# adamchang2000/DenseFusion

Measured on AMD Instinct MI355X. Metric: poses/sec (node) YCB-Video 1000 pts + 2 refine iters, higher is better.
Workload: dtype f32

## Files before the change

densefusion_amd/_lib.py:

```python
from __future__ import annotations

import ctypes
import os

_HERE = os.path.dirname(os.path.abspath(__file__))
LIB_PATH = os.path.join(_HERE, "libdfusion_hip_dev.so" if os.environ.get("DF_DEV_LIB") else "libdfusion_hip.so")
_lib = None

_vp, _i, _i64, _f, _sz = ctypes.c_void_p, ctypes.c_int, ctypes.c_int64, ctypes.c_float, ctypes.c_size_t

class ConvDesc(ctypes.Structure):
    _fields_ = ([(n, ctypes.c_void_p) for n in ("in_", "wgt", "bias", "res", "prelu", "out")] +
                [(n, ctypes.c_int32) for n in ("B", "H", "W", "Cin", "in_ld", "in_coff", "OH", "OW", "Cout", "out_ld",
                                               "out_coff", "res_ld", "res_coff", "KH", "KW", "stride", "pad", "dil",
                                               "act")] +
                [("splitk_ws", ctypes.c_void_p), ("splitk_ws_bytes", ctypes.c_size_t)])


SIGNATURES = {
    "df_last_error": (ctypes.c_char_p, []),
    "df_version": (_i, []),
    "df_knn_device": (_i, [_vp, _i, _vp, _i, _i, _i, _vp, _vp]),
    "df_knn": (_i, [_vp, _vp, _vp, _i, _i, _i, _i, _i, _vp]),
    "knn_device": (None, [_vp, _i, _vp, _i, _i, _i, _vp, _vp, _vp]),
# ... 55 lines not shown
    "df_trainer_flat_numel": (_i64, [_vp]),
    "df_trainer_num_params": (_i, [_vp]),
    "df_trainer_param_info": (_i, [_vp, _i, ctypes.c_char_p, _i, ctypes.POINTER(_i64), ctypes.POINTER(_i)]),
    "df_trainer_pack_param": (_i, [_vp, ctypes.c_char_p, _vp, _vp, _vp]),
    "df_trainer_unpack_param": (_i, [_vp, ctypes.c_char_p, _vp, _vp, _vp]),
    "df_posenet_train_workspace_bytes": (_sz, [_vp, _i, _i, _i, _i]),
    "df_posenet_train_step": (_i, [_vp, _vp, _vp, _i64, _i, _i, _i] + [_vp] * 6 + [_i, _vp, _f, _i, ctypes.c_uint] + [_vp] * 9 + [_sz, _vp]),
    "df_posenet_train_multi_workspace_bytes": (_sz, [_vp, _i, _vp, _vp, _vp, _i]),
    "df_posenet_train_step_multi": (_i, [_vp, _vp, _vp, _i64, _i, _vp, _vp, _vp, _vp] + [_vp] * 5 + [_i, _vp, _f, _i, ctypes.c_uint] + [_vp] * 9 + [_sz, _vp]),
    "df_trainer_set_splitk": (_i, [_vp, _i]),
    "df_trainer_profile": (_i, [_vp, _i]),
    "df_trainer_profile_read": (_i, [_vp, ctypes.POINTER(ctypes.c_double), ctypes.POINTER(ctypes.c_double), ctypes.POINTER(_i)]),
    "df_refiner_train_workspace_bytes": (_sz, [_vp, _i, _i]),
    "df_refiner_train_step": (_i, [_vp, _vp, _vp, _i64, _i] + [_vp] * 5 + [_i, _vp] + [_vp] * 4 + [_sz, _vp]),
    "df_conv3x3_winograd_tile_scratch_bytes": (ctypes.c_size_t, [ctypes.POINTER(ConvDesc), _i]),
    "df_conv3x3_winograd_tile_nhwc": (_i, [ctypes.POINTER(ConvDesc), _i, _vp, ctypes.c_size_t, _vp]),
    "df_conv2d_dgrad_nhwc": (_i, [ctypes.POINTER(ConvDesc), _vp, _vp, _vp, _i, _vp]),
    "df_conv2d_wgrad_workspace_bytes": (ctypes.c_size_t, [ctypes.POINTER(ConvDesc)]),
    "df_conv2d_wgrad_nhwc": (_i, [ctypes.POINTER(ConvDesc), _vp, _vp, _vp, _vp, ctypes.c_size_t, _vp]),
    "df_net_debug_taps": (_i, [_vp, _i]),
    "df_net_debug_tap_read": (_i, [_vp, ctypes.c_char_p, _vp, _i64, ctypes.POINTER(_i64)]),
    "df_net_profile": (_i, [_vp, _i]),
    "df_net_profile_read": (_i, [_vp] + [ctypes.POINTER(ctypes.c_double)] * 4 + [ctypes.POINTER(_i)]),
}


def lib():
    global _lib
    if _lib is None:
        if not os.path.exists(LIB_PATH):
            raise RuntimeError(
                f"{LIB_PATH} not found: the HIP extension is not built. Run "
                "`python -c 'import __graft_entry__ as g; g.build()'` at the repo root (needs hipcc). "
                "densefusion_amd has no CPU fallback.")
        L = ctypes.CDLL(LIB_PATH)
        for name, (res, args) in SIGNATURES.items():
            fn = getattr(L, name)
            fn.restype, fn.argtypes = res, args
        _lib = L
    return _lib


def check(status: int, what: str = "") -> None:
    if status != 0:
        msg = lib().df_last_error().decode("utf-8", "replace")
        raise RuntimeError(f"libdfusion_hip {what} failed ({status}): {msg}")
# ... 36 lines not shown
```

densefusion_amd/csrc/engine.hip:

```cpp
#include <cstdlib>
#include <cstring>
#include <map>
#include <string>
#include <vector>

#include "igemm.h"
#include "layers.h"
#include "wino.h"
#include "pose.h"

namespace df {

struct ParamInfo {
  std::string key;
  int64_t shape[4];
  int ndim;
  int64_t numel() const { int64_t n = 1; for (int i = 0; i < ndim; ++i) n *= shape[i]; return n; }
};

struct Net {
  int kind = 0;
  int num_points = 0, num_obj = 0;
  std::vector<ParamInfo> spec;
  std::map<std::string, int> index;
  std::vector<char> loaded;
  std::map<std::string, float *> buf;
  int device = 0;
  bool profiling = false;
  std::vector<hipEvent_t> ev;
  std::vector<double> ev_flops, ev_bytes, ev_useful;
  std::vector<std::string> ev_desc;
  size_t ev_used = 0;
  bool psp_dirty = false;
  bool upload_pending = false;
  float *stage = nullptr;
  size_t stage_cap = 0;
  bool taps_on = false;
  struct Tap { float *buf = nullptr; size_t cap = 0; int64_t shape[4] = {0, 0, 0, 0}; };
  std::map<std::string, Tap> taps;
};

static void add(Net &n, const std::string &key, std::initializer_list<int64_t> shp) {
  ParamInfo p;
  p.key = key;
  p.ndim = (int)shp.size();
  int i = 0;
  for (auto v : shp) p.shape[i++] = v;
  for (; i < 4; ++i) p.shape[i] = 1;
  n.index[key] = (int)n.spec.size();
  n.spec.push_back(p);
}

static const char *CNN = "cnn.model.module.";

static void build_posenet_spec(Net &n) {
// ... 175 lines not shown
    const std::string nm = std::string("fc") + std::to_string(l);
    if (ends_with(key, ".weight")) e = copy(dev_alloc(n, nm + ".w", (size_t)2 * co * ci) + (size_t)h * co * ci, src, (size_t)co * ci);
    else e = copy(dev_alloc(n, nm + ".bias", 2 * co) + h * co, src, co);
  } else {
    float *dst = dev_alloc(n, key, (size_t)numel);
    if (!dst) return set_error(DF_ERR_LAUNCH, "load_param: hipMalloc failed");
    e = copy(dst, src, (size_t)numel);
  }
  if (e == hipSuccess && n.kind == 1 && key == "feat.conv5.weight") {
    const float *w5 = n.buf[key];
    float *wx = dev_alloc(n, "feat.conv5.wx", (size_t)512 * 192), *we = dev_alloc(n, "feat.conv5.we", (size_t)512 * 192);
    if (!wx || !we) return set_error(DF_ERR_LAUNCH, "load_param: hipMalloc failed");
    e = copy2d(wx, 192, w5, 384, 64, 512);
    if (e == hipSuccess) e = copy2d(wx + 64, 192, w5 + 128, 384, 128, 512);
    if (e == hipSuccess) e = copy2d(we, 192, w5 + 64, 384, 64, 512);
    if (e == hipSuccess) e = copy2d(we + 64, 192, w5 + 256, 384, 128, 512);
  }
  if (e != hipSuccess) return set_error(DF_ERR_LAUNCH, "load_param(%s): %s", key.c_str(), hipGetErrorString(e));
  n.loaded[it->second] = 1;
  if (n.kind == 0 && key.find(".psp.") != std::string::npos && !ends_with(key, ".bias")) n.psp_dirty = true;
  return DF_OK;
}

static int ensure_derived(Net &n) {
  if (!n.psp_dirty) {
    if (n.upload_pending) {
      if (hipStreamSynchronize(0) != hipSuccess) return set_error(DF_ERR_LAUNCH, "parameter upload failed: %s", hipGetErrorString(hipGetLastError()));
      n.upload_pending = false;
    }
    return DF_OK;
  }
  const std::string P = CNN;
  float *wc = dev_alloc(n, "psp.fold.w", (size_t)4 * 1024 * 512), *wf = dev_alloc(n, "psp.fold.wfeat", (size_t)1024 * 512);
  if (!wc || !wf) return set_error(DF_ERR_LAUNCH, "psp fold: hipMalloc failed");
  const float *wb = n.buf[P + "psp.bottleneck.weight"];
  hipMemcpy2DAsync(wf, 512 * sizeof(float), wb + 2048, 2560 * sizeof(float), 512 * sizeof(float), 1024, hipMemcpyDeviceToDevice, 0);
  for (int st = 0; st < 4; ++st)
    hipLaunchKernelGGL(psp_fold_kernel, dim3(2, 1024, 1), dim3(256), 0, 0, wb, n.buf[P + "psp.stages." + std::to_string(st) + ".1.weight"], wc, st);
  if (hipStreamSynchronize(0) != hipSuccess || check_launch("psp fold") != DF_OK) return DF_ERR_LAUNCH;
  n.psp_dirty = false;
  n.upload_pending = false;
  return DF_OK;
}

static int check_ready(const Net &n0) {
  Net &n = const_cast<Net &>(n0);
  for (size_t i = 0; i < n.spec.size(); ++i)
    if (!n.loaded[i]) return set_error(DF_ERR_STATE, "parameter '%s' was never loaded", n.spec[i].key.c_str());
  return ensure_derived(n);
}

struct Ctx {
  Net *net;
  hipStream_t st;
  bool dry;
  char *base;
  size_t off = 0, cap = 0, peak = 0;
  int err = DF_OK;

  float *f(size_t floats) { return reinterpret_cast<float *>(bytes(floats * sizeof(float))); }
  void *bytes(size_t b) {
    b = (b + 255) & ~size_t(255);
    void *p = dry ? nullptr : base + off;
    off += b;
    if (off > peak) peak = off;
// ... 15 lines not shown
    const size_t n = (size_t)d0 * d1 * d2 * d3;
    if (t.cap < n) {
      if (t.buf) hipFree(t.buf);
      t.buf = nullptr; t.cap = 0;
      if (hipMalloc(&t.buf, n * sizeof(float)) != hipSuccess) { (void)hipGetLastError(); return; }
      t.cap = n;
    }
    t.shape[0] = d0; t.shape[1] = d1; t.shape[2] = d2; t.shape[3] = d3;
    hipMemcpyAsync(t.buf, src, n * sizeof(float), hipMemcpyDeviceToDevice, st);
  }
  double pt_useful = 1.0;
  void pconv(const ConvParams &p) { conv(p, pt_useful); }
  void conv(const ConvParams &p, double useful = 1.0) {
    if (!live()) return;
    Net &n = *net;
    if (n.profiling) {
      if (n.ev_used + 2 > n.ev.size()) {
        const size_t old = n.ev.size();
        n.ev.resize(old + 256);
        for (size_t i = old; i < n.ev.size(); ++i) hipEventCreate(&n.ev[i]);
      }
      hipEventRecord(n.ev[n.ev_used], st);
    }
#ifdef DF_DEV
    ConvParams pc = p;
    pc.wgt_const = true;
    const int rc = launch_conv(pc, st);
#else
    const int rc = launch_conv(p, st);
#endif
    if (n.profiling) {
      hipEventRecord(n.ev[n.ev_used + 1], st);
      n.ev_flops.push_back(conv_flops(p));
      n.ev_bytes.push_back(conv_bytes(p));
      n.ev_useful.push_back(conv_flops(p) * useful);
      char d[160];
      snprintf(d, sizeof(d), "M=%ld N=%d K=%d k%dx%d s%d d%d z%d", (long)p.B * p.OH * p.OW, p.Cout, p.KH * p.KW * p.Cin, p.KH,
               p.KW, p.stride, p.dil, p.zcount);
      n.ev_desc.push_back(d);
      n.ev_used += 2;
    }
    if (rc != DF_OK) err = rc;
  }
};

static ConvParams point_gemm(const float *in, int in_ld, int in_coff, int cin, const float *w, const float *bias,
                             float *out, int out_ld, int out_coff, int cout, int rows, int act);

static bool point_fused() {
  static const bool on = df::dev_getenv("DF_POINT_UNFUSED") == nullptr;
  return on;
}

static int wino_route_for(int H, int W, int dil, int ci, int co) {
  static const bool off = df::dev_getenv("DF_NO_WINOGRAD") != nullptr;
  static const int force = df::dev_getenv("DF_WINOGRAD_TILE") ? atoi(df::dev_getenv("DF_WINOGRAD_TILE")) : 0;
  if (off) return 0;
  const int r = wino_route(H, W, dil, ci, co);
  return (r && force == 2) ? 2 : r;
}

static ConvParams point_gemm(const float *in, int in_ld, int in_coff, int cin, const float *w, const float *bias,
// ... 369 lines not shown
extern "C" df_net *df_posenet_create(int num_points, int num_obj) {
  if (num_points <= 0 || num_obj <= 0) { set_error(DF_ERR_ARG, "posenet_create: bad sizes"); return nullptr; }
  Net *n = new Net();
  n->kind = 0; n->num_points = num_points; n->num_obj = num_obj;
  hipGetDevice(&n->device);
  build_posenet_spec(*n);
  n->loaded.assign(n->spec.size(), 0);
  return reinterpret_cast<df_net *>(n);
}

extern "C" df_net *df_refiner_create(int num_points, int num_obj) {
  if (num_points <= 0 || num_obj <= 0) { set_error(DF_ERR_ARG, "refiner_create: bad sizes"); return nullptr; }
  Net *n = new Net();
  n->kind = 1; n->num_points = num_points; n->num_obj = num_obj;
  hipGetDevice(&n->device);
  build_refiner_spec(*n);
  n->loaded.assign(n->spec.size(), 0);
  return reinterpret_cast<df_net *>(n);
}

extern "C" void df_net_destroy(df_net *h) {
  if (!h) return;
  Net *n = as_net(h);
#ifdef DF_DEV
  split_gemm_invalidate();
#endif
  for (auto &kv : n->buf) hipFree(kv.second);
  if (n->stage) hipFree(n->stage);
  for (auto &kv : n->taps) if (kv.second.buf) hipFree(kv.second.buf);
  for (auto e : n->ev) hipEventDestroy(e);
  delete n;
}

extern "C" int df_net_num_params(const df_net *h) { return h ? (int)as_net(h)->spec.size() : 0; }

extern "C" int df_net_param_info(const df_net *h, int i, char *key_out, int key_cap, int64_t *shape4, int *ndim) {
  if (!h) return set_error(DF_ERR_ARG, "param_info: null handle");
  const Net *n = as_net(h);
  if (i < 0 || i >= (int)n->spec.size()) return set_error(DF_ERR_ARG, "param_info: index out of range");
  const ParamInfo &p = n->spec[i];
  if (key_out && key_cap > 0) { strncpy(key_out, p.key.c_str(), key_cap - 1); key_out[key_cap - 1] = 0; }
  if (shape4) for (int d = 0; d < 4; ++d) shape4[d] = p.shape[d];
  if (ndim) *ndim = p.ndim;
  return DF_OK;
}

extern "C" int df_net_load_param(df_net *h, const char *key, const float *ptr, int64_t numel) {
  if (!h || !key) return set_error(DF_ERR_ARG, "load_param: null handle/key");
#ifdef DF_DEV
  split_gemm_invalidate();
#endif
  return load_param(*as_net(h), key, ptr, numel);
}

extern "C" int df_net_profile(df_net *h, int enable) {
  if (!h) return set_error(DF_ERR_ARG, "profile: null handle");
  Net *n = as_net(h);
  n->profiling = enable != 0;
  n->ev_used = 0;
  n->ev_flops.clear();
  n->ev_bytes.clear();
  n->ev_useful.clear();
  n->ev_desc.clear();
  return DF_OK;
}

extern "C" int df_net_profile_read(df_net *h, double *gemm_ms, double *gemm_flops, double *gemm_useful_flops, double *gemm_bytes,
                                   int *launches) {
  if (!h) return set_error(DF_ERR_ARG, "profile_read: null handle");
  Net *n = as_net(h);
  double ms = 0, fl = 0, by = 0, us = 0;
  static const bool verbose = df::dev_getenv("DF_PROFILE_VERBOSE") != nullptr;
  for (size_t i = 0; i + 1 < n->ev_used; i += 2) {
    float t = 0;
    if (hipEventElapsedTime(&t, n->ev[i], n->ev[i + 1]) != hipSuccess) return set_error(DF_ERR_LAUNCH, "profile_read: events not complete");
    ms += t;
    fl += n->ev_flops[i / 2];
    by += n->ev_bytes[i / 2];
    us += n->ev_useful[i / 2];
    if (verbose)
      fprintf(stderr, "[df-gemm] %s  %.1f us  %.1f TFLOP/s\n", n->ev_desc[i / 2].c_str(), t * 1e3, n->ev_flops[i / 2] / t / 1e9);
  }
  if (gemm_ms) *gemm_ms = ms;
  if (gemm_flops) *gemm_flops = fl;
  if (gemm_useful_flops) *gemm_useful_flops = us;
  if (gemm_bytes) *gemm_bytes = by;
  if (launches) *launches = (int)(n->ev_used / 2);
  n->ev_used = 0;
  n->ev_flops.clear();
  n->ev_bytes.clear();
  n->ev_useful.clear();
  n->ev_desc.clear();
  return DF_OK;
}

extern "C" int df_net_debug_taps(df_net *h, int enable) {
  if (!h) return set_error(DF_ERR_ARG, "debug_taps: null handle");
  Net *n = as_net(h);
  n->taps_on = enable != 0;
  if (!enable) {
    for (auto &kv : n->taps) if (kv.second.buf) hipFree(kv.second.buf);
    n->taps.clear();
  }
  return DF_OK;
}

extern "C" int df_net_debug_tap_read(df_net *h, const char *name, float *dst, int64_t cap, int64_t *shape4) {
  if (!h || !name) return set_error(DF_ERR_ARG, "debug_tap_read: null handle / name");
  Net *n = as_net(h);
  auto it = n->taps.find(name);
  if (it == n->taps.end() || !it->second.buf) return set_error(DF_ERR_STATE, "debug_tap_read: no tap named '%s' (arm df_net_debug_taps and run a single-bucket forward)", name);
  const Net::Tap &t = it->second;
  const int64_t numel = t.shape[0] * t.shape[1] * t.shape[2] * t.shape[3];
  if (shape4) for (int i = 0; i < 4; ++i) shape4[i] = t.shape[i];
  if (!dst) return DF_OK;
  if (cap < numel) return set_error(DF_ERR_ARG, "debug_tap_read: destination holds %lld floats, tap '%s' has %lld", (long long)cap, name, (long long)numel);
  if (hipMemcpy(dst, t.buf, (size_t)numel * sizeof(float), hipMemcpyDefault) != hipSuccess) return set_error(DF_ERR_LAUNCH, "debug_tap_read: copy failed");
// ... 355 lines not shown
```

densefusion_amd/csrc/igemm.h:

```cpp
#pragma once
#include "common.h"

namespace df {

enum Act { ACT_NONE = 0, ACT_RELU = 1, ACT_PRELU = 2 };

struct ConvParams {
  const float *in = nullptr;
  const float *wgt = nullptr;
  const float *bias = nullptr;
  const float *res = nullptr;
  const float *prelu = nullptr;
  float *out = nullptr;
  float *colsum = nullptr;
  int B = 1, H = 1, W = 1, Cin = 0, in_ld = 0, in_coff = 0;
  int OH = 1, OW = 1, Cout = 0, out_ld = 0, out_coff = 0;
  int res_ld = 0, res_coff = 0;
  int KH = 1, KW = 1, stride = 1, pad = 0, dil = 1;
  int up = 1;
  int act = ACT_NONE;
  int rows_per_group = 0, rows_valid = 0, bias_group_ld = 0;
  int zcount = 1;
  int ngroup = 0;
  long z_in_coff = 0, z_wgt = 0, z_bias = 0, z_out_coff = 0;
  bool wgt_const = false;
  float *splitk_ws = nullptr;
  size_t splitk_ws_bytes = 0;
  int splitk = 1;
  int tiles_m = 0, tile_gn = 0, tile_full = 0;
  unsigned full_magic = 0, gn_magic = 0, gl_magic = 0, rpg_magic = 0;
  int full_sh = 0, gn_sh = 0, gl_sh = 0, rpg_sh = 0;
  unsigned ohw_magic = 0, ow_magic = 0;
  int ohw_sh = 0, ow_sh = 0;
};

int conv_colsum_rows(const ConvParams &p);
double conv_flops(const ConvParams &p);
double conv_bytes(const ConvParams &p);
int launch_conv(const ConvParams &p, hipStream_t st, int *splitk_used = nullptr);

struct WgradSeg { int B, H, W, OH, OW; long in_row0, out_row0; };
constexpr int CONV_MAX_BUCKETS = 16;
int launch_conv_multi(const ConvParams &p, int nseg, const WgradSeg *segs, hipStream_t st);

size_t wgrad_workspace_bytes(const ConvParams &p);
int launch_wgrad(const ConvParams &p, float *dw, float *db, void *ws, size_t ws_bytes, hipStream_t st, int accumulate = 0);

constexpr int WGRAD_MAX_SEGS = 32;
size_t wgrad_multi_workspace_bytes(const ConvParams &p, int nseg, const WgradSeg *segs);
int launch_wgrad_multi(const ConvParams &p, int nseg, const WgradSeg *segs, float *dw, float *db, void *ws, size_t ws_bytes, hipStream_t st,
                       int accumulate = 0);

#ifdef DF_DEV
int try_split_gemm(const ConvParams &p, hipStream_t st);
void split_gemm_invalidate();
#endif

}
```

densefusion_amd/csrc/igemm.hip:

```cpp
#include <cstdlib>

#include "igemm.h"
#include <algorithm>
#include <type_traits>

#ifndef DF_WTRACE
#define DF_WTRACE(i)
#endif
#ifndef DF_TRACE
#define DF_TRACE(i)
#define DF_TRACE_WAVE_END(w)
#endif

namespace df {
namespace {

typedef float f32x16 __attribute__((ext_vector_type(16)));
typedef float f32x4 __attribute__((ext_vector_type(4)));

constexpr int BK = 32;
constexpr int LDK = 36;

typedef unsigned int u32x4 __attribute__((ext_vector_type(4)));

// ... 1157 lines not shown
  if (ca <= cb && ca <= cc) return {128, 128, 2};
  if (cb <= cc) return {128, 64, 2};
  return {64, 64, 2};
}

}

int conv_colsum_rows(const ConvParams &p) {
  const TileCfg c = pick_cfg(p);
  const long M = (long)p.B * p.OH * p.OW;
  return (int)(((M + c.bm - 1) / c.bm) * c.wmv) * p.zcount;
}

double conv_bytes(const ConvParams &p) {
  const double M = (double)p.B * p.OH * p.OW;
  double b = (double)p.B * p.H * p.W * p.Cin + (double)p.Cout * p.KH * p.KW * p.Cin + (p.out ? M * p.Cout : 0.0) + (p.res ? M * p.Cout : 0.0);
  return b * p.zcount * sizeof(float);
}

double conv_flops(const ConvParams &p) {
  return 2.0 * p.B * p.OH * p.OW * (double)p.Cout * p.KH * p.KW * p.Cin * p.zcount;
}

int launch_conv(const ConvParams &p, hipStream_t st, int *splitk_used) {
  if (!p.in || !p.wgt || (!p.out && !p.colsum)) return set_error(DF_ERR_ARG, "conv: null pointer");
  if (p.Cin % 4 || p.in_ld % 4 || p.in_coff % 4 || p.z_in_coff % 4 || p.z_wgt % 4)
    return set_error(DF_ERR_ARG, "conv: Cin/in_ld/in_coff must be multiples of 4 (16-B vector loads)");
  if (p.KH * p.KW > 1 && (p.Cin & (p.Cin - 1)))
    return set_error(DF_ERR_ARG, "conv: multi-tap convolutions need a power-of-two Cin (got %d)", p.Cin);
  const long M = (long)p.B * p.OH * p.OW;
  if (M <= 0 || p.Cout <= 0) return DF_OK;
  if (M * (long)p.out_ld >= (1L << 40) || (long)p.B * p.H * p.W >= (1L << 31))
    return set_error(DF_ERR_ARG, "conv: tensor too large for 32-bit pixel indexing");
#ifdef DF_DEV
  if (!p.splitk_ws) {
    const int taken = try_split_gemm(p, st);
    if (taken < 0) return taken;
    if (taken) {
      if (splitk_used) *splitk_used = 1;
      return check_launch("split gemm");
    }
  }
#endif
  const TileCfg c = pick_cfg(p);
  ConvParams pl = p;
  make_fdiv((long)p.OH * p.OW, pl.ohw_magic, pl.ohw_sh);
  make_fdiv(p.OW, pl.ow_magic, pl.ow_sh);
  auto set_tile_decode = [&]() {
    const int tiles_n = (p.Cout + c.bn - 1) / c.bn;
    pl.tiles_m = (int)((M + c.bm - 1) / c.bm);
    pl.tile_gn = pl.ngroup > 0 && pl.ngroup < tiles_n ? pl.ngroup : tiles_n;
    pl.tile_full = pl.tiles_m * pl.tile_gn;
    const int last = tiles_n % pl.tile_gn;
    make_fdiv(pl.tile_full, pl.full_magic, pl.full_sh);
    make_fdiv(pl.tile_gn, pl.gn_magic, pl.gn_sh);
    make_fdiv(last ? last : pl.tile_gn, pl.gl_magic, pl.gl_sh);
    make_fdiv(p.rows_per_group > 0 ? p.rows_per_group : 1, pl.rpg_magic, pl.rpg_sh);
  };
  {
    const size_t slice = (size_t)c.bn * p.KH * p.KW * p.Cin * sizeof(float);
    const long tn = (p.Cout + c.bn - 1) / c.bn;
    static const long budget = df::dev_getenv("DF_IGEMM_WGROUP_KB") ? atol(df::dev_getenv("DF_IGEMM_WGROUP_KB")) * 1024L : 3L << 20;
    if (budget > 0 && (size_t)tn * slice > (size_t)budget) pl.ngroup = (int)std::max<long>(1, budget / (long)slice);
  }
  set_tile_decode();
  if (p.rows_per_group > 0 && (p.rows_per_group % c.bm))
// ... 296 lines not shown
```

densefusion_amd/csrc/split_gemm.hip:

```cpp
#include "igemm.h"
#ifdef DF_DEV
#include <map>
#include <mutex>
#include <tuple>

namespace df {
namespace {

typedef __bf16 bf16x8 __attribute__((ext_vector_type(8)));
typedef __bf16 bf16x2 __attribute__((ext_vector_type(2)));
typedef float f32x16 __attribute__((ext_vector_type(16)));
typedef float f32x2 __attribute__((ext_vector_type(2)));

constexpr int SBM = 128, SBN = 128, SBK = 32;
constexpr int PLANE_BYTES = 128 * 64;

__device__ __forceinline__ void cut3(float a0, float a1, unsigned &hi, unsigned &mid, unsigned &lo) {
  const bf16x2 h = __builtin_convertvector(f32x2{a0, a1}, bf16x2);
  hi = __builtin_bit_cast(unsigned, h);
  const float r0 = a0 - __builtin_bit_cast(float, hi << 16), r1 = a1 - __builtin_bit_cast(float, hi & 0xFFFF0000u);
  const bf16x2 m = __builtin_convertvector(f32x2{r0, r1}, bf16x2);
  mid = __builtin_bit_cast(unsigned, m);
  const float s0 = r0 - __builtin_bit_cast(float, mid << 16), s1 = r1 - __builtin_bit_cast(float, mid & 0xFFFF0000u);
  const bf16x2 l = __builtin_convertvector(f32x2{s0, s1}, bf16x2);
  lo = __builtin_bit_cast(unsigned, l);
}

__global__ void cut_weights_kernel(const float *__restrict__ w, unsigned *__restrict__ planes, long pairs) {
  const long i = (long)blockIdx.x * blockDim.x + threadIdx.x;
  if (i >= pairs) return;
  const float2 v = reinterpret_cast<const float2 *>(w)[i];
  unsigned h, m, l;
  cut3(v.x, v.y, h, m, l);
  planes[i] = h; planes[pairs + i] = m; planes[2 * pairs + i] = l;
}

struct SplitArgs {
  const float *in; const __bf16 *wpl; const float *bias; const float *res; const float *prelu; float *out; float *colsum;
  long M, wplane;
  int N, K, in_ld, in_coff, out_ld, out_coff, res_ld, res_coff, act, rows_per_group, rows_valid, bias_group_ld;
  long z_in_coff, z_wgt, z_bias, z_out_coff;
  int tiles_m, tiles_n;
  long cs_rows;
};

__device__ __forceinline__ int piece(int row, int slot) { return row * 64 + ((slot ^ ((row >> 2) & 3)) << 4); }

__device__ __forceinline__ void split_epilogue(const SplitArgs &a, const f32x16 (&acc)[2][2], int z, long row0, int wrow, int nb, int fr, int fh, long cs_row) {
  const float slope = a.act == ACT_PRELU ? a.prelu[0] : 0.f;
  float *out = a.out + z * a.z_out_coff + a.out_coff;
  const float *bias = a.bias ? a.bias + z * a.z_bias : nullptr;
  const float *gbias = bias && a.bias_group_ld > 0 ? bias + (row0 / a.rows_per_group) * a.bias_group_ld : nullptr;
  const int grp = a.rows_per_group > 0 ? (int)(row0 / a.rows_per_group) : 0;
  const long left = a.M - row0;
  const int valid = a.rows_per_group > 0 ? a.rows_valid - (int)(row0 - (long)grp * a.rows_per_group) : (1 << 30);
  const int limit = (int)(left < valid ? left : valid);
#pragma unroll
// ... 251 lines not shown
      if (g >= 8 && g < 32 && (g & 1) == 0) __builtin_amdgcn_sched_group_barrier(0x100, 1, 0); \
      if (g % 5 == 4) __builtin_amdgcn_sched_group_barrier(0x200, 1, 0);         \
    }                                                                            \
    __syncthreads();                                                             \
  } while (0)

  unsigned char *const st0 = lds2, *const st1 = lds2 + V2_STAGE;
  const int nk = a.K / SBK;
  const int klast = a.K - SBK;
  V2_FETCH(x, 0);
  V2_FETCH(y, SBK < klast ? SBK : klast);
  V2_STAGE_TO(x, st0);
  __syncthreads();
  int kt = 0;
  for (; kt + 1 < nk; kt += 2) {
    const int k2 = (kt + 2) * SBK, k3 = (kt + 3) * SBK;
    V2_BODY(x, y, k2 < klast ? k2 : klast, st0, st1);
    V2_BODY(y, x, k3 < klast ? k3 : klast, st1, st0);
  }
  if (nk & 1) { V2_COMPUTE(st0); }
  split_epilogue(a, acc, z, row0, wr * 64, n0 + wc * 64, fr, fh, (long)tm * 4 + wr);
}

struct Planes { __bf16 *ptr; long plane; long epoch; };
std::mutex g_mu;
long g_epoch = 1;
std::map<std::tuple<const float *, long, int>, Planes> g_cache;
std::map<std::tuple<int, hipStream_t>, Planes> g_scratch;

void cut(const float *w, __bf16 *planes, long elems, hipStream_t st) {
  const long pairs = elems / 2;
  hipLaunchKernelGGL(cut_weights_kernel, dim3((unsigned)((pairs + 255) / 256)), dim3(256), 0, st, w, reinterpret_cast<unsigned *>(planes), pairs);
}

Planes weight_planes(const float *w, long elems, bool constant, hipStream_t st) {
  int dev = 0;
  (void)hipGetDevice(&dev);
  std::lock_guard<std::mutex> g(g_mu);
  if (!constant) {
    Planes &sc = g_scratch[std::make_tuple(dev, st)];
    if (sc.plane < elems) {
      if (sc.ptr) (void)hipFree(sc.ptr);
      sc = Planes{nullptr, 0, 0};
      if (hipMalloc(reinterpret_cast<void **>(&sc.ptr), (size_t)elems * 3 * sizeof(__bf16)) != hipSuccess) return Planes{nullptr, 0, 0};
      sc.plane = elems;
    }
    cut(w, sc.ptr, elems, st);
    return Planes{sc.ptr, elems, 0};
  }
  Planes &pl = g_cache[std::make_tuple(w, elems, dev)];
  if (!pl.ptr) {
    if (hipMalloc(reinterpret_cast<void **>(&pl.ptr), (size_t)elems * 3 * sizeof(__bf16)) != hipSuccess) return Planes{nullptr, 0, 0};
    pl.plane = elems;
    pl.epoch = 0;
  }
  if (pl.epoch != g_epoch) {
    cut(w, pl.ptr, elems, st);
    pl.epoch = g_epoch;
  }
  return pl;
}

}

void split_gemm_invalidate() {
  std::lock_guard<std::mutex> g(g_mu);
  ++g_epoch;
}

int try_split_gemm(const ConvParams &p, hipStream_t st) {
  static const bool on = dev_getenv("DF_GEMM_SPLIT_BF16") != nullptr;
  static const bool verbose = dev_getenv("DF_GEMM_SPLIT_VERBOSE") != nullptr;
  if (!on) return 0;
  const long M = (long)p.B * p.OH * p.OW;
  const int K = p.Cin;
  const bool ok = p.KH == 1 && p.KW == 1 && p.stride == 1 && p.pad == 0 && p.up == 1 && p.H == p.OH && p.W == p.OW && (p.out || p.colsum) && !(p.colsum && p.res) && p.splitk <= 1 &&
                  p.Cout % SBN == 0 && K % SBK == 0 && K >= SBK && M >= 1 && (p.rows_per_group == 0 ? p.bias_group_ld == 0 : p.rows_per_group % SBM == 0) && (p.z_wgt % 2) == 0;
  if (verbose) fprintf(stderr, "[df-split] M=%ld N=%d K=%d z%d -> %s\n", M, p.Cout, K, p.zcount, ok ? "bf16 x 6" : "fp32");
  if (!ok) return 0;
  const long elems = (long)(p.zcount - 1) * p.z_wgt + (long)p.Cout * K;
  const Planes pl = weight_planes(p.wgt, elems, p.wgt_const, st);
  if (!pl.ptr) return 0;
  SplitArgs a{};
  a.in = p.in; a.wpl = pl.ptr; a.bias = p.bias; a.res = p.res; a.prelu = p.prelu; a.out = p.out; a.colsum = p.colsum;
  a.M = M; a.wplane = pl.plane; a.N = p.Cout; a.K = K; a.in_ld = p.in_ld; a.in_coff = p.in_coff; a.out_ld = p.out_ld; a.out_coff = p.out_coff;
  a.res_ld = p.res_ld; a.res_coff = p.res_coff; a.act = p.act; a.rows_per_group = p.rows_per_group; a.rows_valid = p.rows_valid; a.bias_group_ld = p.bias_group_ld;
  a.z_in_coff = p.z_in_coff; a.z_wgt = p.z_wgt; a.z_bias = p.z_bias; a.z_out_coff = p.z_out_coff;
  a.cs_rows = ((M + 127) / 128) * 2;
  a.tiles_n = p.Cout / SBN;
  static const int variant = dev_getenv("DF_GEMM_SPLIT_V") ? atoi(dev_getenv("DF_GEMM_SPLIT_V")) : 2;
  const bool v2 = variant == 2 && K >= 384 && (p.rows_per_group == 0 || p.rows_per_group % 256 == 0);
  if (v2) {
    const int rc = raise_lds_limit(reinterpret_cast<const void *>(&gemm_split_bf16_v2_kernel), 2 * V2_STAGE);
    if (rc != DF_OK) return rc;
    a.tiles_m = (int)((M + 255) / 256);
    const unsigned grid = (unsigned)(((a.tiles_m + 7) / 8) * 8 * a.tiles_n);
    hipLaunchKernelGGL(gemm_split_bf16_v2_kernel, dim3(grid, 1, p.zcount), dim3(512), 2 * V2_STAGE, st, a);
  } else {
    a.tiles_m = (int)((M + SBM - 1) / SBM);
    const unsigned grid = (unsigned)(((a.tiles_m + 7) / 8) * 8 * a.tiles_n);
    hipLaunchKernelGGL(gemm_split_bf16_kernel, dim3(grid, 1, p.zcount), dim3(256), 0, st, a);
  }
  return 1;
}

}
#endif
```

include/dfusion.h:

```cpp
#ifndef DFUSION_H_
#define DFUSION_H_

#include <stddef.h>
#include <stdint.h>

#ifdef __cplusplus
extern "C" {
#endif

typedef void *df_stream_t;

#define DF_OK 0
#define DF_ERR_ARG (-1)
#define DF_ERR_LAUNCH (-2)
#define DF_ERR_WORKSPACE (-3)
#define DF_ERR_STATE (-4)

const char *df_last_error(void);
int df_version(void);

#define DF_KNN_MAX_K 32
int df_knn_device(const float *ref_dev, int ref_nb, const float *query_dev, int query_nb, int dim, int k,
                  int64_t *ind_dev, df_stream_t stream);

// ... 140 lines not shown
                          const float *img, const float *cloud, const int64_t *choose, const int64_t *obj, const float *target,
                          const float *model_points, int M, const int *symmetric_host, float w, int dropout, unsigned seed,
                          float *loss_out, float *dis_out, float *new_points, float *new_target, float *out_r, float *out_t,
                          float *out_c, float *emb, void *ws, size_t ws_bytes, df_stream_t stream);
size_t df_posenet_train_multi_workspace_bytes(const df_trainer *t, int nb, const int *B, const int *H, const int *W, int M);
int df_posenet_train_step_multi(df_trainer *t, const float *flat_param, float *flat_grad, int64_t param_version, int nb, const int *B,
                                const int *H, const int *W, const float *const *img, const float *cloud, const int64_t *choose,
                                const int64_t *obj, const float *target, const float *model_points, int M, const int *symmetric_host,
                                float w, int dropout, unsigned seed, float *loss_out, float *dis_out, float *new_points,
                                float *new_target, float *out_r, float *out_t, float *out_c, float *emb, void *ws, size_t ws_bytes,
                                df_stream_t stream);
int df_trainer_set_splitk(df_trainer *t, int enable);
int df_trainer_profile(df_trainer *t, int enable);
int df_trainer_profile_read(df_trainer *t, double *ms3, double *flops3, int *launches3);
size_t df_refiner_train_workspace_bytes(const df_trainer *t, int B, int M);
int df_refiner_train_step(df_trainer *t, const float *flat_param, float *flat_grad, int64_t param_version, int B, const float *points,
                          const float *emb, const int64_t *obj, const float *target, const float *model_points, int M,
                          const int *symmetric_host, float *dis_out, float *new_points, float *new_target, void *ws, size_t ws_bytes,
                          df_stream_t stream);

int df_net_profile(df_net *net, int enable);
int df_net_profile_read(df_net *net, double *gemm_ms, double *gemm_flops, double *gemm_useful_flops, double *gemm_bytes,
                        int *launches);

int df_net_debug_taps(df_net *net, int enable);
int df_net_debug_tap_read(df_net *net, const char *name, float *dst, int64_t cap, int64_t *shape4);

#ifdef __cplusplus
}
#endif
#endif
```

Baseline: 8801.

## Enable split-bf16 GEMM path by default with precut per-net weight planes

Promotes the dev-only split-bf16 (3-plane, 6-product) matrix-core GEMM path to production for 1x1 convs with K>=384 and a supported epilogue. Weights are cut into bf16 hi/mid/lo planes once per parameter load and stored per net, so the forward pass does no per-call cutting. Routed launches fail with an error if the planes are missing. This trades extra weight memory and a more complex routing path for running the large fp32 GEMMs on bf16 matrix cores while keeping near-fp32 accuracy.

```diff
diff --git a/densefusion_amd/_lib.py b/densefusion_amd/_lib.py
--- a/densefusion_amd/_lib.py
+++ b/densefusion_amd/_lib.py
@@ -101,6 +101,8 @@
     "df_net_debug_tap_read": (_i, [_vp, ctypes.c_char_p, _vp, _i64, ctypes.POINTER(_i64)]),
     "df_net_profile": (_i, [_vp, _i]),
     "df_net_profile_read": (_i, [_vp] + [ctypes.POINTER(ctypes.c_double)] * 4 + [ctypes.POINTER(_i)]),
+    "df_net_profile_read_split": (_i, [_vp] + [ctypes.POINTER(ctypes.c_double)] * 3 + [ctypes.POINTER(_i)]),
+    "df_gemm_route": (_i, [_i, _i, _i]),
 }
 
 
diff --git a/densefusion_amd/csrc/engine.hip b/densefusion_amd/csrc/engine.hip
--- a/densefusion_amd/csrc/engine.hip
+++ b/densefusion_amd/csrc/engine.hip
@@ -30,7 +30,11 @@
   std::vector<hipEvent_t> ev;
   std::vector<double> ev_flops, ev_bytes, ev_useful;
   std::vector<std::string> ev_desc;
+  std::vector<char> ev_bf16;
   size_t ev_used = 0;
+  struct Planes { long elems = 0, stride = 0; void *ptr = nullptr; };
+  std::map<const float *, Planes> planes;
+  bool planes_dirty = true;
   bool psp_dirty = false;
   bool upload_pending = false;
   float *stage = nullptr;
@@ -252,8 +256,94 @@
   return DF_OK;
 }
 
+struct GemmWeight { std::string name; int N, K, epi; };
+static std::vector<GemmWeight> gemm_weights(const Net &n) {
+  std::vector<GemmWeight> v;
+  const std::string P = CNN;
+  if (n.kind == 0) {
+    v.push_back({"psp.fold.w", 1024, 512, GEMM_EPI_PLAIN});
+    v.push_back({"psp.fold.wfeat", 1024, 512, GEMM_EPI_RESIDUAL});
+    v.push_back({P + "up_1.conv.1.weight.tm", 9 * 256, 1024, GEMM_EPI_PLAIN});
+    v.push_back({P + "up_2.conv.1.weight.tm", 9 * 64, 256, GEMM_EPI_PLAIN});
+    v.push_back({P + "up_3.conv.1.weight", 64, 576, GEMM_EPI_PLAIN});
+    for (const ParamInfo &pi : n.spec)
+      if (pi.key.find("feats.layer") != std::string::npos && pi.ndim == 4) {
+        const int O = (int)pi.shape[0], I = (int)pi.shape[1];
+        if (pi.shape[2] * pi.shape[3] == 1) v.push_back({pi.key, O, I, GEMM_EPI_PLAIN});
+        else {
+          v.push_back({pi.key + ".wino", O, I, GEMM_EPI_PLAIN});
+          v.push_back({pi.key + ".wino4", O, I, GEMM_EPI_PLAIN});
+        }
+      }
+    v.push_back({"feat.conv5.weight", 512, 256, GEMM_EPI_PLAIN});
+    v.push_back({"head1.wpt", 1920, 384, GEMM_EPI_GROUPS});
+    v.push_back({"head1.wpt", 640, 384, GEMM_EPI_GROUPS});
+    v.push_back({"head2.w", 256, 640, GEMM_EPI_PLAIN});
+    v.push_back({"head3.w", 128, 256, GEMM_EPI_PLAIN});
+  } else {
+    v.push_back({"feat.conv5.we", 512, 192, GEMM_EPI_PLAIN});
+    v.push_back({"feat.conv5.wx", 512, 192, GEMM_EPI_RESIDUAL});
+  }
+  v.push_back({"feat.e_conv1.weight", 64, 32, GEMM_EPI_PLAIN});
+  v.push_back({"feat.conv2.weight", 128, 64, GEMM_EPI_PLAIN});
+  v.push_back({"feat.e_conv2.weight", 128, 64, GEMM_EPI_PLAIN});
+  v.push_back({"feat.conv6.weight", 1024, 512, GEMM_EPI_GROUPS});
+  return v;
+}
+
+static long buffer_elems(const Net &n, const std::string &name) {
+  const std::string P = CNN;
+  auto spec_of = [&](const std::string &key) -> const ParamInfo * {
+    auto it = n.index.find(key);
+    return it == n.index.end() ? nullptr : &n.spec[it->second];
+  };
+  if (name == "psp.fold.w") return 4L * 1024 * 512;
+  if (name == "psp.fold.wfeat") return 1024L * 512;
+  if (name == "head1.wpt") return 1920L * 384;
+  if (name == "head2.w") return 3L * 256 * 640;
+  if (name == "head3.w") return 3L * 128 * 256;
+  if (name == "feat.conv5.we" || name == "feat.conv5.wx") return 512L * 192;
+  const bool wino = ends_with(name, ".wino"), wino4 = ends_with(name, ".wino4"), tm = ends_with(name, ".tm");
+  const std::string key = wino ? name.substr(0, name.size() - 5) : wino4 ? name.substr(0, name.size() - 6) : tm ? name.substr(0, name.size() - 3) : name;
+  const ParamInfo *pi = spec_of(key);
+  if (!pi) return 0;
+  const long O = pi->shape[0], I = pi->shape[1], HW = pi->ndim == 4 ? pi->shape[2] * pi->shape[3] : 1;
+  if (wino) return 16 * O * I;
+  if (wino4) return 36 * O * I;
+  if (tm) return 9 * O * I;
+  return O * HW * ((I + 3) / 4 * 4);
+}
+
+static int cut_planes(Net &n) {
+  for (const GemmWeight &g : gemm_weights(n)) {
+    if (!split_route(g.N, g.K, g.epi)) continue;
+    auto it = n.buf.find(g.name);
+    const long elems = buffer_elems(n, g.name);
+    if (it == n.buf.end() || elems <= 0) return set_error(DF_ERR_STATE, "weight planes: no packed buffer '%s'", g.name.c_str());
+    Net::Planes &pl = n.planes[it->second];
+    if (!pl.ptr) {
+      pl.elems = elems;
+      pl.stride = (elems + 63) / 64 * 64;
+      if (hipMalloc(&pl.ptr, (size_t)pl.stride * 3 * 2) != hipSuccess) {
+        pl.ptr = nullptr;
+        return set_error(DF_ERR_LAUNCH, "weight planes of '%s': hipMalloc failed", g.name.c_str());
+      }
+      hipMemset(pl.ptr, 0, (size_t)pl.stride * 3 * 2);
+    }
+    cut_weight_planes(it->second, pl.ptr, pl.elems, pl.stride, 0);
+  }
+  if (check_launch("weight planes") != DF_OK) return DF_ERR_LAUNCH;
+  return DF_OK;
+}
+
 static int ensure_derived(Net &n) {
   if (!n.psp_dirty) {
+    if (n.planes_dirty) {
+      const int rc = cut_planes(n);
+      if (rc != DF_OK) return rc;
+      n.planes_dirty = false;
+      n.upload_pending = true;
+    }
     if (n.upload_pending) {
       if (hipStreamSynchronize(0) != hipSuccess) return set_error(DF_ERR_LAUNCH, "parameter upload failed: %s", hipGetErrorString(hipGetLastError()));
       n.upload_pending = false;
@@ -267,10 +357,10 @@
   hipMemcpy2DAsync(wf, 512 * sizeof(float), wb + 2048, 2560 * sizeof(float), 512 * sizeof(float), 1024, hipMemcpyDeviceToDevice, 0);
   for (int st = 0; st < 4; ++st)
     hipLaunchKernelGGL(psp_fold_kernel, dim3(2, 1024, 1), dim3(256), 0, 0, wb, n.buf[P + "psp.stages." + std::to_string(st) + ".1.weight"], wc, st);
-  if (hipStreamSynchronize(0) != hipSuccess || check_launch("psp fold") != DF_OK) return DF_ERR_LAUNCH;
+  if (check_launch("psp fold") != DF_OK) return DF_ERR_LAUNCH;
   n.psp_dirty = false;
-  n.upload_pending = false;
-  return DF_OK;
+  n.upload_pending = true;
+  return ensure_derived(n);
 }
 
 static int check_ready(const Net &n0) {
@@ -332,13 +422,24 @@
       }
       hipEventRecord(n.ev[n.ev_used], st);
     }
-#ifdef DF_DEV
     ConvParams pc = p;
-    pc.wgt_const = true;
-    const int rc = launch_conv(pc, st);
-#else
-    const int rc = launch_conv(p, st);
-#endif
+    if (p.KH * p.KW == 1 && split_route(p.Cout, p.Cin, gemm_epi_kind(p))) {
+      const long extent = (long)(p.zcount - 1) * p.z_wgt + (long)p.Cout * p.Cin;
+      auto it = n.planes.upper_bound(p.wgt);
+      const Net::Planes *pl = nullptr;
+      if (it != n.planes.begin()) {
+        --it;
+        if (p.wgt >= it->first && p.wgt + extent <= it->first + it->second.elems && (p.wgt - it->first) % 8 == 0) pl = &it->second;
+      }
+      if (!pl) {
+        if (err == DF_OK) err = set_error(DF_ERR_STATE, "routed GEMM N=%d K=%d: its weights have no bf16 planes", p.Cout, p.Cin);
+        return;
+      }
+      pc.wpl = reinterpret_cast<const char *>(pl->ptr) + (p.wgt - it->first) * 2;
+      pc.wpl_stride = pl->stride;
+    }
+    int on_bf16 = 0;
+    const int rc = launch_conv(pc, st, nullptr, &on_bf16);
     if (n.profiling) {
       hipEventRecord(n.ev[n.ev_used + 1], st);
       n.ev_flops.push_back(conv_flops(p));
@@ -348,6 +449,7 @@
       snprintf(d, sizeof(d), "M=%ld N=%d K=%d k%dx%d s%d d%d z%d", (long)p.B * p.OH * p.OW, p.Cout, p.KH * p.KW * p.Cin, p.KH,
                p.KW, p.stride, p.dil, p.zcount);
       n.ev_desc.push_back(d);
+      n.ev_bf16.push_back((char)on_bf16);
       n.ev_used += 2;
     }
     if (rc != DF_OK) err = rc;
@@ -763,9 +865,7 @@
 extern "C" void df_net_destroy(df_net *h) {
   if (!h) return;
   Net *n = as_net(h);
-#ifdef DF_DEV
-  split_gemm_invalidate();
-#endif
+  for (auto &kv : n->planes) hipFree(kv.second.ptr);
   for (auto &kv : n->buf) hipFree(kv.second);
   if (n->stage) hipFree(n->stage);
   for (auto &kv : n->taps) if (kv.second.buf) hipFree(kv.second.buf);
@@ -788,9 +888,7 @@
 
 extern "C" int df_net_load_param(df_net *h, const char *key, const float *ptr, int64_t numel) {
   if (!h || !key) return set_error(DF_ERR_ARG, "load_param: null handle/key");
-#ifdef DF_DEV
-  split_gemm_invalidate();
-#endif
+  as_net(h)->planes_dirty = true;
   return load_param(*as_net(h), key, ptr, numel);
 }
 
@@ -803,6 +901,7 @@
   n->ev_bytes.clear();
   n->ev_useful.clear();
   n->ev_desc.clear();
+  n->ev_bf16.clear();
   return DF_OK;
 }
 
@@ -811,10 +910,15 @@
   if (!h) return set_error(DF_ERR_ARG, "profile_read: null handle");
   Net *n = as_net(h);
   double ms = 0, fl = 0, by = 0, us = 0;
+  int cnt = 0;
   static const bool verbose = df::dev_getenv("DF_PROFILE_VERBOSE") != nullptr;
   for (size_t i = 0; i + 1 < n->ev_used; i += 2) {
     float t = 0;
     if (hipEventElapsedTime(&t, n->ev[i], n->ev[i + 1]) != hipSuccess) return set_error(DF_ERR_LAUNCH, "profile_read: events not complete");
+    if (verbose && n->ev_bf16[i / 2])
+      fprintf(stderr, "[df-gemm-bf16] %s  %.1f us  %.1f TFLOP/s\n", n->ev_desc[i / 2].c_str(), t * 1e3, n->ev_flops[i / 2] / t / 1e9);
+    if (n->ev_bf16[i / 2]) continue;
+    ++cnt;
     ms += t;
     fl += n->ev_flops[i / 2];
     by += n->ev_bytes[i / 2];
@@ -826,14 +930,38 @@
   if (gemm_flops) *gemm_flops = fl;
   if (gemm_useful_flops) *gemm_useful_flops = us;
   if (gemm_bytes) *gemm_bytes = by;
-  if (launches) *launches = (int)(n->ev_used / 2);
+  if (launches) *launches = cnt;
   n->ev_used = 0;
   n->ev_flops.clear();
   n->ev_bytes.clear();
   n->ev_useful.clear();
   n->ev_desc.clear();
+  n->ev_bf16.clear();
   return DF_OK;
 }
+
+extern "C" int df_net_profile_read_split(df_net *h, double *gemm_ms, double *gemm_flops, double *gemm_useful_flops, int *launches) {
+  if (!h) return set_error(DF_ERR_ARG, "profile_read_split: null handle");
+  Net *n = as_net(h);
+  double ms = 0, fl = 0, us = 0;
+  int cnt = 0;
+  for (size_t i = 0; i + 1 < n->ev_used; i += 2) {
+    if (!n->ev_bf16[i / 2]) continue;
+    float t = 0;
+    if (hipEventElapsedTime(&t, n->ev[i], n->ev[i + 1]) != hipSuccess) return set_error(DF_ERR_LAUNCH, "profile_read_split: events not complete");
+    ms += t;
+    fl += n->ev_flops[i / 2];
+    us += n->ev_useful[i / 2];
+    ++cnt;
+  }
+  if (gemm_ms) *gemm_ms = ms;
+  if (gemm_flops) *gemm_flops = fl;
+  if (gemm_useful_flops) *gemm_useful_flops = us;
+  if (launches) *launches = cnt;
+  return DF_OK;
+}
+
+extern "C" int df_gemm_route(int n, int k, int epilogue) { return split_route(n, k, epilogue); }
 
 extern "C" int df_net_debug_taps(df_net *h, int enable) {
   if (!h) return set_error(DF_ERR_ARG, "debug_taps: null handle");
diff --git a/densefusion_amd/csrc/igemm.h b/densefusion_amd/csrc/igemm.h
--- a/densefusion_amd/csrc/igemm.h
+++ b/densefusion_amd/csrc/igemm.h
@@ -23,7 +23,8 @@
   int zcount = 1;
   int ngroup = 0;
   long z_in_coff = 0, z_wgt = 0, z_bias = 0, z_out_coff = 0;
-  bool wgt_const = false;
+  const void *wpl = nullptr;
+  long wpl_stride = 0;
   float *splitk_ws = nullptr;
   size_t splitk_ws_bytes = 0;
   int splitk = 1;
@@ -37,7 +38,7 @@
 int conv_colsum_rows(const ConvParams &p);
 double conv_flops(const ConvParams &p);
 double conv_bytes(const ConvParams &p);
-int launch_conv(const ConvParams &p, hipStream_t st, int *splitk_used = nullptr);
+int launch_conv(const ConvParams &p, hipStream_t st, int *splitk_used = nullptr, int *on_bf16 = nullptr);
 
 struct WgradSeg { int B, H, W, OH, OW; long in_row0, out_row0; };
 constexpr int CONV_MAX_BUCKETS = 16;
@@ -51,9 +52,10 @@
 int launch_wgrad_multi(const ConvParams &p, int nseg, const WgradSeg *segs, float *dw, float *db, void *ws, size_t ws_bytes, hipStream_t st,
                        int accumulate = 0);
 
-#ifdef DF_DEV
+enum GemmEpi { GEMM_EPI_PLAIN = 0, GEMM_EPI_RESIDUAL = 1, GEMM_EPI_GROUPS = 2, GEMM_EPI_OTHER = 3 };
+int gemm_epi_kind(const ConvParams &p);
+int split_route(int N, int K, int epi);
+void cut_weight_planes(const float *w, void *planes, long elems, long stride, hipStream_t st);
 int try_split_gemm(const ConvParams &p, hipStream_t st);
-void split_gemm_invalidate();
-#endif
 
 }
diff --git a/densefusion_amd/csrc/igemm.hip b/densefusion_amd/csrc/igemm.hip
--- a/densefusion_amd/csrc/igemm.hip
+++ b/densefusion_amd/csrc/igemm.hip
@@ -1203,7 +1203,8 @@
   return 2.0 * p.B * p.OH * p.OW * (double)p.Cout * p.KH * p.KW * p.Cin * p.zcount;
 }
 
-int launch_conv(const ConvParams &p, hipStream_t st, int *splitk_used) {
+int launch_conv(const ConvParams &p, hipStream_t st, int *splitk_used, int *on_bf16) {
+  if (on_bf16) *on_bf16 = 0;
   if (!p.in || !p.wgt || (!p.out && !p.colsum)) return set_error(DF_ERR_ARG, "conv: null pointer");
   if (p.Cin % 4 || p.in_ld % 4 || p.in_coff % 4 || p.z_in_coff % 4 || p.z_wgt % 4)
     return set_error(DF_ERR_ARG, "conv: Cin/in_ld/in_coff must be multiples of 4 (16-B vector loads)");
@@ -1213,16 +1214,15 @@
   if (M <= 0 || p.Cout <= 0) return DF_OK;
   if (M * (long)p.out_ld >= (1L << 40) || (long)p.B * p.H * p.W >= (1L << 31))
     return set_error(DF_ERR_ARG, "conv: tensor too large for 32-bit pixel indexing");
-#ifdef DF_DEV
-  if (!p.splitk_ws) {
+  {
     const int taken = try_split_gemm(p, st);
     if (taken < 0) return taken;
     if (taken) {
       if (splitk_used) *splitk_used = 1;
+      if (on_bf16) *on_bf16 = 1;
       return check_launch("split gemm");
     }
   }
-#endif
   const TileCfg c = pick_cfg(p);
   ConvParams pl = p;
   make_fdiv((long)p.OH * p.OW, pl.ohw_magic, pl.ohw_sh);
diff --git a/densefusion_amd/csrc/split_gemm.hip b/densefusion_amd/csrc/split_gemm.hip
--- a/densefusion_amd/csrc/split_gemm.hip
+++ b/densefusion_amd/csrc/split_gemm.hip
@@ -3,6 +3,7 @@
 #include <map>
 #include <mutex>
 #include <tuple>
+#endif
 
 namespace df {
 namespace {
@@ -26,13 +27,13 @@
   lo = __builtin_bit_cast(unsigned, l);
 }
 
-__global__ void cut_weights_kernel(const float *__restrict__ w, unsigned *__restrict__ planes, long pairs) {
+__global__ void cut_planes_kernel(const float *__restrict__ w, __bf16 *__restrict__ planes, long elems, long stride) {
   const long i = (long)blockIdx.x * blockDim.x + threadIdx.x;
-  if (i >= pairs) return;
-  const float2 v = reinterpret_cast<const float2 *>(w)[i];
+  if (i >= elems) return;
   unsigned h, m, l;
-  cut3(v.x, v.y, h, m, l);
-  planes[i] = h; planes[pairs + i] = m; planes[2 * pairs + i] = l;
+  cut3(w[i], 0.f, h, m, l);
+  unsigned short *pl = reinterpret_cast<unsigned short *>(planes);
+  pl[i] = (unsigned short)h; pl[stride + i] = (unsigned short)m; pl[2 * stride + i] = (unsigned short)l;
 }
 
 struct SplitArgs {
@@ -330,68 +331,71 @@
   split_epilogue(a, acc, z, row0, wr * 64, n0 + wc * 64, fr, fh, (long)tm * 4 + wr);
 }
 
-struct Planes { __bf16 *ptr; long plane; long epoch; };
+#ifdef DF_DEV
 std::mutex g_mu;
-long g_epoch = 1;
-std::map<std::tuple<const float *, long, int>, Planes> g_cache;
-std::map<std::tuple<int, hipStream_t>, Planes> g_scratch;
-
-void cut(const float *w, __bf16 *planes, long elems, hipStream_t st) {
-  const long pairs = elems / 2;
-  hipLaunchKernelGGL(cut_weights_kernel, dim3((unsigned)((pairs + 255) / 256)), dim3(256), 0, st, w, reinterpret_cast<unsigned *>(planes), pairs);
-}
-
-Planes weight_planes(const float *w, long elems, bool constant, hipStream_t st) {
+std::map<std::tuple<int, hipStream_t>, std::pair<__bf16 *, long>> g_scratch;
+
+const __bf16 *scratch_planes(const float *w, long elems, hipStream_t st) {
   int dev = 0;
   (void)hipGetDevice(&dev);
   std::lock_guard<std::mutex> g(g_mu);
-  if (!constant) {
-    Planes &sc = g_scratch[std::make_tuple(dev, st)];
-    if (sc.plane < elems) {
-      if (sc.ptr) (void)hipFree(sc.ptr);
-      sc = Planes{nullptr, 0, 0};
-      if (hipMalloc(reinterpret_cast<void **>(&sc.ptr), (size_t)elems * 3 * sizeof(__bf16)) != hipSuccess) return Planes{nullptr, 0, 0};
-      sc.plane = elems;
-    }
-    cut(w, sc.ptr, elems, st);
-    return Planes{sc.ptr, elems, 0};
-  }
-  Planes &pl = g_cache[std::make_tuple(w, elems, dev)];
-  if (!pl.ptr) {
-    if (hipMalloc(reinterpret_cast<void **>(&pl.ptr), (size_t)elems * 3 * sizeof(__bf16)) != hipSuccess) return Planes{nullptr, 0, 0};
-    pl.plane = elems;
-    pl.epoch = 0;
-  }
-  if (pl.epoch != g_epoch) {
-    cut(w, pl.ptr, elems, st);
-    pl.epoch = g_epoch;
-  }
-  return pl;
-}
-
-}
-
-void split_gemm_invalidate() {
-  std::lock_guard<std::mutex> g(g_mu);
-  ++g_epoch;
+  auto &sc = g_scratch[std::make_tuple(dev, st)];
+  if (sc.second < elems) {
+    if (sc.first) (void)hipFree(sc.first);
+    sc = {nullptr, 0};
+    if (hipMalloc(reinterpret_cast<void **>(&sc.first), (size_t)elems * 3 * sizeof(__bf16)) != hipSuccess) return nullptr;
+    sc.second = elems;
+  }
+  cut_weight_planes(w, sc.first, elems, elems, st);
+  return sc.first;
+}
+#endif
+
+}
+
+int split_route(int N, int K, int epi) {
+  if (N <= 0 || N % SBN != 0 || K % SBK != 0 || K < 384) return 0;
+  return epi == GEMM_EPI_PLAIN || epi == GEMM_EPI_RESIDUAL || epi == GEMM_EPI_GROUPS;
+}
+
+int gemm_epi_kind(const ConvParams &p) {
+  const bool groups = p.rows_per_group > 0 || p.bias_group_ld > 0 || p.colsum;
+  if (p.res) return groups ? GEMM_EPI_OTHER : GEMM_EPI_RESIDUAL;
+  return groups ? GEMM_EPI_GROUPS : GEMM_EPI_PLAIN;
+}
+
+void cut_weight_planes(const float *w, void *planes, long elems, long stride, hipStream_t st) {
+  hipLaunchKernelGGL(cut_planes_kernel, dim3((unsigned)((elems + 255) / 256)), dim3(256), 0, st, w, reinterpret_cast<__bf16 *>(planes), elems, stride);
 }
 
 int try_split_gemm(const ConvParams &p, hipStream_t st) {
-  static const bool on = dev_getenv("DF_GEMM_SPLIT_BF16") != nullptr;
+  static const bool off = dev_getenv("DF_GEMM_SPLIT_OFF") != nullptr;
+  static const bool all = dev_getenv("DF_GEMM_SPLIT_BF16") != nullptr;
   static const bool verbose = dev_getenv("DF_GEMM_SPLIT_VERBOSE") != nullptr;
-  if (!on) return 0;
+  if (off || p.splitk_ws || (!p.wpl && !all)) return 0;
   const long M = (long)p.B * p.OH * p.OW;
   const int K = p.Cin;
-  const bool ok = p.KH == 1 && p.KW == 1 && p.stride == 1 && p.pad == 0 && p.up == 1 && p.H == p.OH && p.W == p.OW && (p.out || p.colsum) && !(p.colsum && p.res) && p.splitk <= 1 &&
-                  p.Cout % SBN == 0 && K % SBK == 0 && K >= SBK && M >= 1 && (p.rows_per_group == 0 ? p.bias_group_ld == 0 : p.rows_per_group % SBM == 0) && (p.z_wgt % 2) == 0;
-  if (verbose) fprintf(stderr, "[df-split] M=%ld N=%d K=%d z%d -> %s\n", M, p.Cout, K, p.zcount, ok ? "bf16 x 6" : "fp32");
-  if (!ok) return 0;
-  const long elems = (long)(p.zcount - 1) * p.z_wgt + (long)p.Cout * K;
-  const Planes pl = weight_planes(p.wgt, elems, p.wgt_const, st);
-  if (!pl.ptr) return 0;
+  const bool ok = p.KH == 1 && p.KW == 1 && p.stride == 1 && p.pad == 0 && p.up == 1 && p.H == p.OH && p.W == p.OW && (p.out || p.colsum) &&
+                  p.Cout % SBN == 0 && K % SBK == 0 && K >= SBK && M >= 1 && gemm_epi_kind(p) != GEMM_EPI_OTHER &&
+                  (p.rows_per_group == 0 ? p.bias_group_ld == 0 : p.rows_per_group % SBM == 0) && (p.z_wgt % 8) == 0;
+  const bool take = ok && (all || split_route(p.Cout, K, gemm_epi_kind(p)));
+  if (verbose) fprintf(stderr, "[df-split] M=%ld N=%d K=%d z%d -> %s\n", M, p.Cout, K, p.zcount, take ? "bf16 x 6" : "fp32");
+  if (!take) {
+    if (p.wpl && !all) return set_error(DF_ERR_ARG, "split gemm: routed launch M=%ld N=%d K=%d outside the kernels' cover", M, p.Cout, K);
+    return 0;
+  }
+  const __bf16 *wpl = reinterpret_cast<const __bf16 *>(p.wpl);
+  long wplane = p.wpl_stride;
+#ifdef DF_DEV
+  if (!wpl) {
+    wplane = (long)(p.zcount - 1) * p.z_wgt + (long)p.Cout * K;
+    wpl = scratch_planes(p.wgt, wplane, st);
+    if (!wpl) return set_error(DF_ERR_LAUNCH, "split gemm: hipMalloc of the weight-plane scratch failed");
+  }
+#endif
   SplitArgs a{};
-  a.in = p.in; a.wpl = pl.ptr; a.bias = p.bias; a.res = p.res; a.prelu = p.prelu; a.out = p.out; a.colsum = p.colsum;
-  a.M = M; a.wplane = pl.plane; a.N = p.Cout; a.K = K; a.in_ld = p.in_ld; a.in_coff = p.in_coff; a.out_ld = p.out_ld; a.out_coff = p.out_coff;
+  a.in = p.in; a.wpl = wpl; a.bias = p.bias; a.res = p.res; a.prelu = p.prelu; a.out = p.out; a.colsum = p.colsum;
+  a.M = M; a.wplane = wplane; a.N = p.Cout; a.K = K; a.in_ld = p.in_ld; a.in_coff = p.in_coff; a.out_ld = p.out_ld; a.out_coff = p.out_coff;
   a.res_ld = p.res_ld; a.res_coff = p.res_coff; a.act = p.act; a.rows_per_group = p.rows_per_group; a.rows_valid = p.rows_valid; a.bias_group_ld = p.bias_group_ld;
   a.z_in_coff = p.z_in_coff; a.z_wgt = p.z_wgt; a.z_bias = p.z_bias; a.z_out_coff = p.z_out_coff;
   a.cs_rows = ((M + 127) / 128) * 2;
@@ -413,4 +417,3 @@
 }
 
 }
-#endif
diff --git a/include/dfusion.h b/include/dfusion.h
--- a/include/dfusion.h
+++ b/include/dfusion.h
@@ -186,6 +186,9 @@
 int df_net_profile(df_net *net, int enable);
 int df_net_profile_read(df_net *net, double *gemm_ms, double *gemm_flops, double *gemm_useful_flops, double *gemm_bytes,
                         int *launches);
+int df_net_profile_read_split(df_net *net, double *gemm_ms, double *gemm_flops, double *gemm_useful_flops, int *launches);
+
+int df_gemm_route(int n, int k, int epilogue);
 
 int df_net_debug_taps(df_net *net, int enable);
 int df_net_debug_tap_read(df_net *net, const char *name, float *dst, int64_t cap, int64_t *shape4);
```

Result: faster. 9628, median of 6 (+9.4%).
